# david-zwicker/video-analysis

Hardware: AMD Instinct MI355X
Metric: frames/sec (bg-sub+blur+thresh+CCL) 1080p uint8 (higher is better)
Workload: dtype u8; 1 GPU; cfg3_1080p_full_chain: 1920x1080 uint8, batch 256/GPU, running-mean bg-sub (f64 state) + sigma=5 Gaussian (q8.8) + threshold 20 + 5x5 dilate/erode + 4-connected labelling + object counts; inputs resident in HBM; engine=bg=1 gauss=mfma-i8(ksize=31) thresh=20 morph=2 ccl=4, video=one clip per rank, overlap=off, world_size=1, backend=single process

## Files before the change

### video-analysis_amd/csrc/va_gauss_mfma.hip

```cpp
#include "va_common.h"

namespace va {

namespace {

typedef int v4i __attribute__((ext_vector_type(4)));
typedef int v16i __attribute__((ext_vector_type(16)));
typedef uint32_t u4 __attribute__((ext_vector_type(4)));
typedef u4 u4_unaligned __attribute__((aligned(1)));

constexpr int kWaves = 4;
constexpr int kTileCols = kWaves * 32;
constexpr int kLdsStride = kTileCols + 32 + 16;
static_assert((kLdsStride / 16) % 2 == 1, "LDS row stride must be an odd multiple of 16 bytes");
constexpr int kTapTable = 128;
#ifndef GMF_DST_AUX
#define GMF_DST_AUX 0
#endif
constexpr int kFlushTiles = 8;
constexpr int kFlushRows = 32 * kFlushTiles;
static_assert(kFlushRows == kWaves * 64, "one thread per collected row at a flush");

struct MfmaTaps {
    int ksize;
    int sum;
    int8_t w[36];
};

__device__ __forceinline__ uint32_t bswap32(uint32_t v)
{
    return __builtin_amdgcn_perm(0u, v, 0x00010203u);
}

template <bool HAS_DST, bool HAS_BITS, bool MASK8 = false>
__global__ __launch_bounds__(kWaves * 64, 4) void gauss_mfma_kernel(
    const uint8_t *__restrict__ src, uint8_t *__restrict__ dst, uint32_t *__restrict__ bits,
    int thresh, int h, int w, int w32, int nstrips, int blocks_per_frame, int nframes, MfmaTaps tp,
    int maxval = 255)
{
    __shared__ __attribute__((aligned(16))) uint8_t s_stage[2][32 * kLdsStride];
    __shared__ int8_t s_taps[kTapTable];
    __shared__ __attribute__((aligned(16))) uint32_t s_bits[2][kFlushRows][kWaves];
    constexpr int kDstStride = kTileCols / 4 + 1;
    __shared__ uint32_t s_dst[HAS_DST ? 2 : 1][HAS_DST ? 32 : 1][kDstStride];

    if (threadIdx.x < kTapTable) {
        const int e = (int)threadIdx.x - 48;
        int v = 0;
#pragma unroll
        for (int k = 0; k < 33; k++)
            v = (e == k && k < tp.ksize) ? (int)tp.w[k] : v;
        s_taps[threadIdx.x] = (int8_t)v;
    }
    __syncthreads();

    const int xcd = blockIdx.x & 7, q = blockIdx.x >> 3;
    const int frame = (q / blocks_per_frame) * 8 + xcd;
    const int wave = threadIdx.x >> 6, lane = threadIdx.x & 63;
    const int strip = (q % blocks_per_frame) * kWaves + wave;
    if (frame >= nframes)
        return;
    const bool active = strip < nstrips;

    const int xb = (q % blocks_per_frame) * kTileCols;
    const int R = tp.ksize >> 1;
    const int nn = lane & 31, hh = lane >> 5;
    const int x0 = strip * 32;

    v4i brow[2], bcol[2];
#pragma unroll
    for (int ks = 0; ks < 2; ks++)
#pragma unroll
        for (int g = 0; g < 4; g++) {
            uint32_t wr = 0, wc = 0;
#pragma unroll
            for (int b = 0; b < 4; b++) {
                const int pr = 32 * ks + 16 * hh + 4 * g + b;
                const int pc = 32 * ks + b + 8 * g + 4 * hh;
                const int tr = s_taps[pr - 16 - nn + R + 48];
                const int tc = -(int)s_taps[pc - 16 - nn + R + 48];
                wr |= (uint32_t)(uint8_t)tr << (8 * b);
                wc |= (uint32_t)(uint8_t)tc << (8 * b);
            }
            brow[ks][g] = (int)wr;
            bcol[ks][g] = (int)wc;
        }

    const int k0 = (128 + 128 * tp.sum) * tp.sum;
    const int acc_min = thresh < 0 ? 0 : ((thresh + 1) << 16) - 32768;
    const int c_lo = acc_min - 1 - k0;
    const int k_dst = acc_min - 1 + 32768;

    const uint8_t *fsrc = src + (size_t)frame * h * w;
    const int ntiles = (h + 31) >> 5;

    const int tid = threadIdx.x;
    const int row_a = tid >> 3, ch_a = tid & 7;
    const int row_b = lane >> 1, ch_b = 8 + (lane & 1);
    auto chunk_src = [&](int ch, bool &mir) {
        const int xc = xb - 16 + 16 * ch;
        mir = xc < 0 || xc >= w;
        const int xs = xc < 0 ? -xc - 15 : (xc >= w ? 2 * w - 17 - xc : xc);
        return min(max(xs, 0), w - 16);
    };
    bool mir_a, mir_b;
    const int xs_a = chunk_src(ch_a, mir_a), xs_b = chunk_src(ch_b, mir_b);
    const bool border_block = (xb == 0) || (xb + kTileCols + 16 > w);

    auto row_of = [&](int t, int r) {
        int y = 32 * t - 16 + r;
        y = y < 0 ? -y : y;
        y = y >= h ? 2 * (h - 1) - y : y;
        return min(max(y, 0), h - 1);
    };
    auto fetch = [&](int t, u4 &ga, u4 &gb) {
        const uint8_t *pa, *pb;
        if (t >= 1 && 32 * t + 16 <= h) {
            const uint8_t *base = fsrc + (size_t)(32 * t - 16) * w;
            pa = base + (size_t)row_a * w + xs_a;
            pb = base + (size_t)row_b * w + xs_b;
        } else {
            pa = fsrc + (size_t)row_of(t, row_a) * w + xs_a;
            pb = fsrc + (size_t)row_of(t, row_b) * w + xs_b;
        }
        ga = *reinterpret_cast<const u4_unaligned *>(pa);
        if (wave == 0)
            gb = *reinterpret_cast<const u4_unaligned *>(pb);
    };
    auto stage_write = [&](uint8_t *buf, u4 ga, u4 gb) {
        if (border_block) {
            const u4 ra = {bswap32(ga.w), bswap32(ga.z), bswap32(ga.y), bswap32(ga.x)};
            const u4 rb = {bswap32(gb.w), bswap32(gb.z), bswap32(gb.y), bswap32(gb.x)};
            ga = mir_a ? ra : ga;
            gb = mir_b ? rb : gb;
        }
        *reinterpret_cast<u4 *>(buf + row_a * kLdsStride + 16 * ch_a) = ga ^ 0x80808080u;
        if (wave == 0)
            *reinterpret_cast<u4 *>(buf + row_b * kLdsStride + 16 * ch_b) = gb ^ 0x80808080u;
    };

    v16i c_init;
#pragma unroll
    for (int i = 0; i < 16; i++)
        c_init[i] = c_lo;
    asm volatile("" : "+v"(c_init));

    const uint32_t kOob = 0xFFFFFFFFu;
    __amdgpu_buffer_rsrc_t bits_rsrc = __builtin_amdgcn_make_buffer_rsrc(
        HAS_BITS ? (void *)(bits + (size_t)frame * h * w32) : nullptr, 0, h * w32 * 4, 0x00027000);
    __amdgpu_buffer_rsrc_t dst_rsrc = __builtin_amdgcn_make_buffer_rsrc(
        HAS_DST ? (void *)(dst + (size_t)frame * h * w) : nullptr, 0, h * w, 0x00027000);
    const int xbw = xb >> 5;
    const int valid = max(0, min(32, w - x0));
    const uint32_t colmask = valid < 32 ? (1u << valid) - 1u : ~0u;
    const int frag_off = nn * kLdsStride + 32 * wave + 16 * hh;

    u4 ga, gb = {};
    fetch(0, ga, gb);
    stage_write(s_stage[0], ga, gb);
    fetch(1, ga, gb);
    __syncthreads();
    v4i prev_hi = {}, prev_lo = {};
    v16i yh = {}, yl = {};

    for (int t = 0; t <= ntiles + 1; t++) {
        const uint8_t *cur_buf = s_stage[t & 1];
        uint8_t *next_buf = s_stage[(t + 1) & 1];
        const v4i a0 = *reinterpret_cast<const v4i *>(cur_buf + frag_off);
        const v4i a1 = *reinterpret_cast<const v4i *>(cur_buf + frag_off + 32);
        v16i x = {};
        v4i vout = {};
        if (HAS_DST)
#pragma unroll
            for (int j = 0; j < 4; j++)
                vout[j] = (int)s_dst[(t + 1) & 1][tid >> 3][(tid & 7) * 4 + j];
        x = __builtin_amdgcn_mfma_i32_32x32x32_i8(a0, brow[0], x, 0, 0, 0);
        x = __builtin_amdgcn_mfma_i32_32x32x32_i8(a1, brow[1], x, 0, 0, 0);

        {
            uint32_t p = 0;
            int tv[16];
#pragma unroll
            for (int i = 15; i >= 0; i--) {
                tv[i] = (yh[i] << 8) + yl[i];
                if (HAS_BITS)
                    p = __builtin_amdgcn_alignbit(p, (uint32_t)tv[i], 31);
            }
            const int u = t - 2;
#ifndef GMF_NO_DST_LDS
            if (HAS_DST) {
#pragma unroll
                for (int g = 0; g < 4; g++) {
                    if (MASK8) {
                        const uint32_t t01 = __builtin_amdgcn_perm((uint32_t)tv[4 * g + 1], (uint32_t)tv[4 * g], 0x0c0c0703u);
                        const uint32_t t23 = __builtin_amdgcn_perm((uint32_t)tv[4 * g + 3], (uint32_t)tv[4 * g + 2], 0x07030c0cu);
                        s_dst[u & 1][nn][8 * wave + 2 * g + hh] = (t01 | t23) & (0x01010101u * (uint32_t)maxval);
                    } else {
                        const uint32_t d0 = (uint32_t)(k_dst - tv[4 * g]), d1 = (uint32_t)(k_dst - tv[4 * g + 1]);
                        const uint32_t d2 = (uint32_t)(k_dst - tv[4 * g + 2]), d3 = (uint32_t)(k_dst - tv[4 * g + 3]);
                        s_dst[u & 1][nn][8 * wave + 2 * g + hh] =
                            __builtin_amdgcn_perm(d1, d0, 0x0c0c0602u) | __builtin_amdgcn_perm(d3, d2, 0x06020c0cu);
                    }
                }
            }
#endif
            if (HAS_BITS) {
                uint32_t wd = (p & 0xFu) | ((p & 0xF0u) << 4) | ((p & 0xF00u) << 8) | ((p & 0xF000u) << 12);
                wd <<= 4 * hh;
                const auto sw = __builtin_amdgcn_permlane32_swap(wd, wd, false, false);
                if (hh == 0 && u >= 0)
                    s_bits[(u / kFlushTiles) & 1][(u % kFlushTiles) * 32 + nn][wave] =
                        active ? (wd | sw[1]) & colmask : 0u;
            }
        }

        stage_write(next_buf, ga, gb);
        fetch(min(t + 2, ntiles), ga, gb);
        if (HAS_DST) {
            const int us = t - 3, r = tid >> 3, c16 = (tid & 7) * 16, y = 32 * us + r;
#ifdef GMF_NO_DST_STORE
            const bool ok = false;
#else
            const bool ok = us >= 0 && y < h && xb + c16 < w;
#endif
            __builtin_amdgcn_raw_buffer_store_b128(vout, dst_rsrc, ok ? (uint32_t)(y * w + xb + c16) : kOob, 0, GMF_DST_AUX);
        }

        v4i cur_hi, cur_lo;
#pragma unroll
        for (int g = 0; g < 4; g++) {
            const uint32_t t01 = __builtin_amdgcn_perm((uint32_t)x[4 * g + 1], (uint32_t)x[4 * g], 0x05010400u);
            const uint32_t t23 = __builtin_amdgcn_perm((uint32_t)x[4 * g + 3], (uint32_t)x[4 * g + 2], 0x05010400u);
            cur_lo[g] = (int)(__builtin_amdgcn_perm(t23, t01, 0x05040100u) ^ 0x80808080u);
            cur_hi[g] = (int)__builtin_amdgcn_perm(t23, t01, 0x07060302u);
        }

        yh = __builtin_amdgcn_mfma_i32_32x32x32_i8(prev_hi, bcol[0], v16i{}, 0, 0, 0);
        yl = __builtin_amdgcn_mfma_i32_32x32x32_i8(prev_lo, bcol[0], c_init, 0, 0, 0);
        yh = __builtin_amdgcn_mfma_i32_32x32x32_i8(cur_hi, bcol[1], yh, 0, 0, 0);
        yl = __builtin_amdgcn_mfma_i32_32x32x32_i8(cur_lo, bcol[1], yl, 0, 0, 0);
        prev_hi = cur_hi;
        prev_lo = cur_lo;
        lds_barrier();

        const int u = t - 2;
        if (HAS_BITS && u >= 0 && (u % kFlushTiles == kFlushTiles - 1 || u == ntiles - 1)) {
            const int g = u / kFlushTiles, y = g * kFlushRows + tid;
            const bool ok = y < h && tid < (u % kFlushTiles + 1) * 32;
            const v4i v = *reinterpret_cast<const v4i *>(&s_bits[g & 1][tid][0]);
            const uint32_t off = (uint32_t)(y * w32 + xbw) * 4u;
            if (xbw + kWaves <= w32) {
                __builtin_amdgcn_raw_buffer_store_b128(v, bits_rsrc, ok ? off : kOob, 0, 0);
            } else {
#pragma unroll
                for (int k = 0; k < kWaves; k++)
                    __builtin_amdgcn_raw_buffer_store_b32(v[k], bits_rsrc,
                                                          ok && xbw + k < w32 ? off + 4 * k : kOob, 0, 0);
            }
        }
    }
    if (HAS_DST) {
        const int us = ntiles - 1, r = tid >> 3, c16 = (tid & 7) * 16, y = 32 * us + r;
        const bool ok = y < h && xb + c16 < w;
        v4i v;
#pragma unroll
        for (int j = 0; j < 4; j++)
            v[j] = (int)s_dst[us & 1][r][(tid & 7) * 4 + j];
        __builtin_amdgcn_raw_buffer_store_b128(v, dst_rsrc, ok ? (uint32_t)(y * w + xb + c16) : kOob, 0, 0);
    }
}

}

bool gauss_mfma_supported(int w, int h, const TapsQ8 &taps)
{
    if (w < 64 || h < 32 || (w % 16) != 0)
        return false;
    if (taps.ksize < 3 || taps.ksize / 2 > 16)
        return false;
    int sum = 0;
    for (int i = 0; i < taps.ksize; i++) {
        if (taps.t[i] > 127)
            return false;
        sum += taps.t[i];
    }
    return sum <= 256;
}

int launch_gauss_mfma_u8(const uint8_t *src, uint8_t *dst, uint32_t *bits, int thresh, int n,
                         int h, int w, const TapsQ8 &taps, hipStream_t st, int mask8_maxval)
{
    VA_REQUIRE(src && (dst || bits), "mfma gaussian: no output requested");
    VA_REQUIRE(mask8_maxval <= 0 || (dst && !bits && thresh >= 0 && mask8_maxval <= 255),
               "mfma gaussian: the byte-mask form writes dst only and needs a threshold");
    VA_REQUIRE(gauss_mfma_supported(w, h, taps), "mfma gaussian: unsupported kernel size %d",
               taps.ksize);
    VA_REQUIRE(reinterpret_cast<uintptr_t>(src) % 16 == 0 &&
                   (!dst || reinterpret_cast<uintptr_t>(dst) % 4 == 0),
               "mfma gaussian: the frame buffers must be 16-byte aligned");
    if (n == 0)
        return VA_OK;
    MfmaTaps tp = {};
    tp.ksize = taps.ksize;
    for (int i = 0; i < taps.ksize; i++) {
        tp.w[i] = (int8_t)taps.t[i];
        tp.sum += taps.t[i];
    }
    const int nstrips = cdiv(w, 32), w32 = words_per_row(w);
    const int bpf = cdiv(w, kTileCols);
    dim3 grid((unsigned)(8 * cdiv(n, 8) * bpf));
    if (mask8_maxval > 0)
        gauss_mfma_kernel<true, false, true><<<grid, kWaves * 64, 0, st>>>(src, dst, bits, thresh, h, w, w32, nstrips, bpf, n, tp,
                                                                            mask8_maxval);
    else if (dst && bits)
        gauss_mfma_kernel<true, true><<<grid, kWaves * 64, 0, st>>>(src, dst, bits, thresh, h, w, w32, nstrips, bpf, n, tp);
    else if (dst)
        gauss_mfma_kernel<true, false><<<grid, kWaves * 64, 0, st>>>(src, dst, bits, thresh, h, w, w32, nstrips, bpf, n, tp);
    else
        gauss_mfma_kernel<false, true><<<grid, kWaves * 64, 0, st>>>(src, dst, bits, thresh, h, w, w32, nstrips, bpf, n, tp);
    VA_LAUNCH_CHECK("gauss_mfma_kernel");
    return VA_OK;
}

}
```

Measured before the change: 309,300 frames/s.

## Make MFMA Gaussian kernel persistent, pipelining work items across column strips

Launches only as many workgroups as can be resident (per-device occupancy query, cached) and has each loop over several (frame, column-block) items assigned round-robin per XCD. The tile pipeline continues across item boundaries: the next item's first tiles are fetched while the previous item's last rows are flushed, removing per-block prologue/epilogue and tap-table setup. This costs extra index bookkeeping, per-item buffer-resource rebuilding, and a more intricate wraparound schedule that could mis-order outputs.

```diff
diff --git a/video-analysis_amd/csrc/va_gauss_mfma.hip b/video-analysis_amd/csrc/va_gauss_mfma.hip
--- a/video-analysis_amd/csrc/va_gauss_mfma.hip
+++ b/video-analysis_amd/csrc/va_gauss_mfma.hip
@@ -1,4 +1,7 @@
 #include "va_common.h"
+
+#include <algorithm>
+#include <atomic>
 
 namespace va {
 
@@ -17,6 +20,9 @@
 #ifndef GMF_DST_AUX
 #define GMF_DST_AUX 0
 #endif
+#ifndef GMF_BITS_AUX
+#define GMF_BITS_AUX 0
+#endif
 constexpr int kFlushTiles = 8;
 constexpr int kFlushRows = 32 * kFlushTiles;
 static_assert(kFlushRows == kWaves * 64, "one thread per collected row at a flush");
@@ -44,6 +50,18 @@
     constexpr int kDstStride = kTileCols / 4 + 1;
     __shared__ uint32_t s_dst[HAS_DST ? 2 : 1][HAS_DST ? 32 : 1][kDstStride];
 
+    const int xcd = blockIdx.x & 7, q = blockIdx.x >> 3, slots = gridDim.x >> 3;
+    const int nitems = xcd < nframes ? ((nframes - xcd + 7) >> 3) * blocks_per_frame : 0;
+    if (q >= nitems)
+        return;
+    const int cnt = (nitems - q + slots - 1) / slots;
+    auto item_at = [&](int k, int &frame, int &xb) {
+        const int j = q + min(k, cnt - 1) * slots;
+        const int fl = j / blocks_per_frame;
+        frame = fl * 8 + xcd;
+        xb = (j - fl * blocks_per_frame) * kTileCols;
+    };
+
     if (threadIdx.x < kTapTable) {
         const int e = (int)threadIdx.x - 48;
         int v = 0;
@@ -54,18 +72,10 @@
     }
     __syncthreads();
 
-    const int xcd = blockIdx.x & 7, q = blockIdx.x >> 3;
-    const int frame = (q / blocks_per_frame) * 8 + xcd;
     const int wave = threadIdx.x >> 6, lane = threadIdx.x & 63;
-    const int strip = (q % blocks_per_frame) * kWaves + wave;
-    if (frame >= nframes)
-        return;
-    const bool active = strip < nstrips;
-
-    const int xb = (q % blocks_per_frame) * kTileCols;
+    const int wave_u = __builtin_amdgcn_readfirstlane(wave);
     const int R = tp.ksize >> 1;
     const int nn = lane & 31, hh = lane >> 5;
-    const int x0 = strip * 32;
 
     v4i brow[2], bcol[2];
 #pragma unroll
@@ -91,21 +101,29 @@
     const int c_lo = acc_min - 1 - k0;
     const int k_dst = acc_min - 1 + 32768;
 
-    const uint8_t *fsrc = src + (size_t)frame * h * w;
     const int ntiles = (h + 31) >> 5;
+    const int T = ntiles + 1;
 
     const int tid = threadIdx.x;
     const int row_a = tid >> 3, ch_a = tid & 7;
     const int row_b = lane >> 1, ch_b = 8 + (lane & 1);
-    auto chunk_src = [&](int ch, bool &mir) {
+    auto chunk_src = [&](int xb, int ch, bool &mir) {
         const int xc = xb - 16 + 16 * ch;
         mir = xc < 0 || xc >= w;
         const int xs = xc < 0 ? -xc - 15 : (xc >= w ? 2 * w - 17 - xc : xc);
         return min(max(xs, 0), w - 16);
     };
-    bool mir_a, mir_b;
-    const int xs_a = chunk_src(ch_a, mir_a), xs_b = chunk_src(ch_b, mir_b);
-    const bool border_block = (xb == 0) || (xb + kTileCols + 16 > w);
+    const uint8_t *fsrc;
+    int xs_a, xs_b;
+    bool mir_a, mir_b, border_block;
+    auto set_fetch_item = [&](int k) {
+        int frame, xb;
+        item_at(k, frame, xb);
+        fsrc = src + (size_t)frame * h * w;
+        xs_a = chunk_src(xb, ch_a, mir_a);
+        xs_b = chunk_src(xb, ch_b, mir_b);
+        border_block = (xb == 0) || (xb + kTileCols + 16 > w);
+    };
 
     auto row_of = [&](int t, int r) {
         int y = 32 * t - 16 + r;
@@ -146,15 +164,25 @@
     asm volatile("" : "+v"(c_init));
 
     const uint32_t kOob = 0xFFFFFFFFu;
-    __amdgpu_buffer_rsrc_t bits_rsrc = __builtin_amdgcn_make_buffer_rsrc(
-        HAS_BITS ? (void *)(bits + (size_t)frame * h * w32) : nullptr, 0, h * w32 * 4, 0x00027000);
-    __amdgpu_buffer_rsrc_t dst_rsrc = __builtin_amdgcn_make_buffer_rsrc(
-        HAS_DST ? (void *)(dst + (size_t)frame * h * w) : nullptr, 0, h * w, 0x00027000);
-    const int xbw = xb >> 5;
-    const int valid = max(0, min(32, w - x0));
-    const uint32_t colmask = valid < 32 ? (1u << valid) - 1u : ~0u;
+    __amdgpu_buffer_rsrc_t bits_rsrc = __builtin_amdgcn_make_buffer_rsrc((void *)bits, 0, 0, 0x00027000);
+    __amdgpu_buffer_rsrc_t dst_rsrc = __builtin_amdgcn_make_buffer_rsrc((void *)dst, 0, 0, 0x00027000);
+    int o_xb = 0;
+    uint32_t colmask = 0;
+    auto set_out_item = [&](int k) {
+        int frame, xb;
+        item_at(k, frame, xb);
+        bits_rsrc = __builtin_amdgcn_make_buffer_rsrc(
+            HAS_BITS ? (void *)(bits + (size_t)frame * h * w32) : nullptr, 0, h * w32 * 4, 0x00027000);
+        dst_rsrc = __builtin_amdgcn_make_buffer_rsrc(
+            HAS_DST ? (void *)(dst + (size_t)frame * h * w) : nullptr, 0, h * w, 0x00027000);
+        o_xb = xb;
+        const int strip = (xb >> 5) + wave_u;
+        const int valid = max(0, min(32, w - strip * 32));
+        colmask = strip < nstrips ? (valid < 32 ? (1u << valid) - 1u : ~0u) : 0u;
+    };
     const int frag_off = nn * kLdsStride + 32 * wave + 16 * hh;
 
+    set_fetch_item(0);
     u4 ga, gb = {};
     fetch(0, ga, gb);
     stage_write(s_stage[0], ga, gb);
@@ -163,9 +191,11 @@
     v4i prev_hi = {}, prev_lo = {};
     v16i yh = {}, yl = {};
 
-    for (int t = 0; t <= ntiles + 1; t++) {
-        const uint8_t *cur_buf = s_stage[t & 1];
-        uint8_t *next_buf = s_stage[(t + 1) & 1];
+    const int total = cnt * T + 2;
+    int s = 0, k = 0;
+    for (int gs = 0; gs < total; gs++) {
+        const uint8_t *cur_buf = s_stage[gs & 1];
+        uint8_t *next_buf = s_stage[(gs + 1) & 1];
         const v4i a0 = *reinterpret_cast<const v4i *>(cur_buf + frag_off);
         const v4i a1 = *reinterpret_cast<const v4i *>(cur_buf + frag_off + 32);
         v16i x = {};
@@ -173,10 +203,11 @@
         if (HAS_DST)
 #pragma unroll
             for (int j = 0; j < 4; j++)
-                vout[j] = (int)s_dst[(t + 1) & 1][tid >> 3][(tid & 7) * 4 + j];
+                vout[j] = (int)s_dst[(gs + 1) & 1][tid >> 3][(tid & 7) * 4 + j];
         x = __builtin_amdgcn_mfma_i32_32x32x32_i8(a0, brow[0], x, 0, 0, 0);
         x = __builtin_amdgcn_mfma_i32_32x32x32_i8(a1, brow[1], x, 0, 0, 0);
 
+        const int u = s >= 2 ? s - 2 : (s == 0 ? ntiles - 1 : -1);
         {
             uint32_t p = 0;
             int tv[16];
@@ -186,7 +217,6 @@
                 if (HAS_BITS)
                     p = __builtin_amdgcn_alignbit(p, (uint32_t)tv[i], 31);
             }
-            const int u = t - 2;
 #ifndef GMF_NO_DST_LDS
             if (HAS_DST) {
 #pragma unroll
@@ -194,11 +224,11 @@
                     if (MASK8) {
                         const uint32_t t01 = __builtin_amdgcn_perm((uint32_t)tv[4 * g + 1], (uint32_t)tv[4 * g], 0x0c0c0703u);
                         const uint32_t t23 = __builtin_amdgcn_perm((uint32_t)tv[4 * g + 3], (uint32_t)tv[4 * g + 2], 0x07030c0cu);
-                        s_dst[u & 1][nn][8 * wave + 2 * g + hh] = (t01 | t23) & (0x01010101u * (uint32_t)maxval);
+                        s_dst[gs & 1][nn][8 * wave + 2 * g + hh] = (t01 | t23) & (0x01010101u * (uint32_t)maxval);
                     } else {
                         const uint32_t d0 = (uint32_t)(k_dst - tv[4 * g]), d1 = (uint32_t)(k_dst - tv[4 * g + 1]);
                         const uint32_t d2 = (uint32_t)(k_dst - tv[4 * g + 2]), d3 = (uint32_t)(k_dst - tv[4 * g + 3]);
-                        s_dst[u & 1][nn][8 * wave + 2 * g + hh] =
+                        s_dst[gs & 1][nn][8 * wave + 2 * g + hh] =
                             __builtin_amdgcn_perm(d1, d0, 0x0c0c0602u) | __builtin_amdgcn_perm(d3, d2, 0x06020c0cu);
                     }
                 }
@@ -209,21 +239,23 @@
                 wd <<= 4 * hh;
                 const auto sw = __builtin_amdgcn_permlane32_swap(wd, wd, false, false);
                 if (hh == 0 && u >= 0)
-                    s_bits[(u / kFlushTiles) & 1][(u % kFlushTiles) * 32 + nn][wave] =
-                        active ? (wd | sw[1]) & colmask : 0u;
+                    s_bits[(u / kFlushTiles) & 1][(u % kFlushTiles) * 32 + nn][wave] = (wd | sw[1]) & colmask;
             }
         }
 
         stage_write(next_buf, ga, gb);
-        fetch(min(t + 2, ntiles), ga, gb);
+        if (s == T - 2)
+            set_fetch_item(k + 1);
+        fetch(s + 2 < T ? s + 2 : s + 2 - T, ga, gb);
         if (HAS_DST) {
-            const int us = t - 3, r = tid >> 3, c16 = (tid & 7) * 16, y = 32 * us + r;
+            const int us = s >= 3 ? s - 3 : (s == 2 ? -1 : ntiles - 2 + s);
+            const int r = tid >> 3, c16 = (tid & 7) * 16, y = 32 * us + r;
 #ifdef GMF_NO_DST_STORE
             const bool ok = false;
 #else
-            const bool ok = us >= 0 && y < h && xb + c16 < w;
+            const bool ok = us >= 0 && y < h && o_xb + c16 < w;
 #endif
-            __builtin_amdgcn_raw_buffer_store_b128(vout, dst_rsrc, ok ? (uint32_t)(y * w + xb + c16) : kOob, 0, GMF_DST_AUX);
+            __builtin_amdgcn_raw_buffer_store_b128(vout, dst_rsrc, ok ? (uint32_t)(y * w + o_xb + c16) : kOob, 0, GMF_DST_AUX);
         }
 
         v4i cur_hi, cur_lo;
@@ -243,31 +275,49 @@
         prev_lo = cur_lo;
         lds_barrier();
 
-        const int u = t - 2;
         if (HAS_BITS && u >= 0 && (u % kFlushTiles == kFlushTiles - 1 || u == ntiles - 1)) {
             const int g = u / kFlushTiles, y = g * kFlushRows + tid;
             const bool ok = y < h && tid < (u % kFlushTiles + 1) * 32;
             const v4i v = *reinterpret_cast<const v4i *>(&s_bits[g & 1][tid][0]);
+            const int xbw = o_xb >> 5;
             const uint32_t off = (uint32_t)(y * w32 + xbw) * 4u;
             if (xbw + kWaves <= w32) {
-                __builtin_amdgcn_raw_buffer_store_b128(v, bits_rsrc, ok ? off : kOob, 0, 0);
+                __builtin_amdgcn_raw_buffer_store_b128(v, bits_rsrc, ok ? off : kOob, 0, GMF_BITS_AUX);
             } else {
 #pragma unroll
-                for (int k = 0; k < kWaves; k++)
-                    __builtin_amdgcn_raw_buffer_store_b32(v[k], bits_rsrc,
-                                                          ok && xbw + k < w32 ? off + 4 * k : kOob, 0, 0);
-            }
-        }
-    }
-    if (HAS_DST) {
-        const int us = ntiles - 1, r = tid >> 3, c16 = (tid & 7) * 16, y = 32 * us + r;
-        const bool ok = y < h && xb + c16 < w;
-        v4i v;
-#pragma unroll
-        for (int j = 0; j < 4; j++)
-            v[j] = (int)s_dst[us & 1][r][(tid & 7) * 4 + j];
-        __builtin_amdgcn_raw_buffer_store_b128(v, dst_rsrc, ok ? (uint32_t)(y * w + xb + c16) : kOob, 0, 0);
-    }
+                for (int k2 = 0; k2 < kWaves; k2++)
+                    __builtin_amdgcn_raw_buffer_store_b32(v[k2], bits_rsrc,
+                                                          ok && xbw + k2 < w32 ? off + 4 * k2 : kOob, 0, GMF_BITS_AUX);
+            }
+        }
+        if (s == 1)
+            set_out_item(k);
+        if (++s == T) {
+            s = 0;
+            k++;
+        }
+    }
+}
+
+constexpr int kMaxDevices = 64;
+template <auto Kernel>
+int resident_workgroups(int *out)
+{
+    static std::atomic<int> cache[kMaxDevices];
+    int dev = 0;
+    VA_HIP(hipGetDevice(&dev));
+    int r = dev >= 0 && dev < kMaxDevices ? cache[dev].load(std::memory_order_relaxed) : 0;
+    if (r == 0) {
+        int per_cu = 0, cus = 0;
+        VA_HIP(hipOccupancyMaxActiveBlocksPerMultiprocessor(&per_cu, Kernel, kWaves * 64, 0));
+        VA_HIP(hipDeviceGetAttribute(&cus, hipDeviceAttributeMultiprocessorCount, dev));
+        VA_REQUIRE(per_cu > 0 && cus > 0, "mfma gaussian: the device holds no workgroup of the kernel");
+        r = per_cu * cus;
+        if (dev >= 0 && dev < kMaxDevices)
+            cache[dev].store(r, std::memory_order_relaxed);
+    }
+    *out = r;
+    return VA_OK;
 }
 
 }
@@ -308,7 +358,15 @@
     }
     const int nstrips = cdiv(w, 32), w32 = words_per_row(w);
     const int bpf = cdiv(w, kTileCols);
-    dim3 grid((unsigned)(8 * cdiv(n, 8) * bpf));
+    int resident = 0;
+    const int rc = mask8_maxval > 0 ? resident_workgroups<gauss_mfma_kernel<true, false, true>>(&resident)
+                   : dst && bits    ? resident_workgroups<gauss_mfma_kernel<true, true>>(&resident)
+                   : dst            ? resident_workgroups<gauss_mfma_kernel<true, false>>(&resident)
+                                    : resident_workgroups<gauss_mfma_kernel<false, true>>(&resident);
+    if (rc != VA_OK)
+        return rc;
+    const long long slots = std::min<long long>(std::max(resident / 8, 1), (long long)cdiv(n, 8) * bpf);
+    dim3 grid((unsigned)(8 * slots));
     if (mask8_maxval > 0)
         gauss_mfma_kernel<true, false, true><<<grid, kWaves * 64, 0, st>>>(src, dst, bits, thresh, h, w, w32, nstrips, bpf, n, tp,
                                                                             mask8_maxval);
```

New measurement: 309,300 frames/s (median of 2 runs). About the same (-0.0%).
